# LeoIV/polyaxon

Hardware: AMD Instinct MI355X
Metric: HPO trials/hour (whole node) + wall-clock-to-target, ResNet-50 Hyperband sweep (higher is better)
Workload: dtype bf16

## Files before the change

polyaxon_amd/csrc/bn_kernels.hip:

```cpp
#include <hip/hip_runtime.h>

#include "handoff.h"
#include <stdint.h>

#define PLX_API extern "C" __attribute__((visibility("default")))

namespace {

constexpr int kBlock = 256;

struct alignas(16) bf16x8 {
  uint16_t v[8];
};

__device__ __forceinline__ float bf2f(uint16_t b) { return __uint_as_float(((uint32_t)b) << 16); }

__device__ __forceinline__ uint16_t f2bf(float f) {
  return __builtin_bit_cast(uint16_t, (__bf16)f);
}

__device__ __forceinline__ void load8(const bf16x8* p, float* f) {
  const bf16x8 v = *p;
#pragma unroll
  for (int k = 0; k < 8; ++k) f[k] = bf2f(v.v[k]);
// ... 865 lines not shown
                                          int64_t M, int C, const float* gamma, const float* save_mean,
                                          const float* save_invstd, float* dgamma, float* dbeta, float* coef,
                                          const float* partials, int nblk, float* l2, int relu, int accumulate,
                                          const ResBn* resbn, unsigned* counters, hipStream_t stream) {
  Plan p;
  if (!plan_for(M, C, &p) || M < 1 || nblk < 1 || (relu && mask == nullptr)) return 1;
  if (resbn != nullptr && (dres == nullptr || resbn->part == nullptr)) return 1;
  const ResBn rb = resbn != nullptr ? *resbn : ResBn{};
  reduce_finalize_bwd(stream, partials, nblk, l2, counters,
                      BwdFin{C, M, gamma, save_mean, save_invstd, dgamma, dbeta, coef, accumulate});
  const int64_t n_vec = M * p.G;
  launch_dx(stream, n_vec, p.G, x, mask, dy, dx, dres, coef, relu, rb);
  return (int)hipGetLastError();
}

PLX_API int plx_stem_bn_pool_forward(const void* x, void* y, void* idx, int N, int H, int W, int C, const float* gamma,
                                     const float* beta, float eps, float momentum, float* running_mean,
                                     float* running_var, float* save_mean, float* save_invstd, float* scale_bias,
                                     float* partials, const float* ext_part, int ext_nblk, unsigned* counters,
                                     hipStream_t stream) {
  const int G = C / 8;
  if (N <= 0 || H <= 0 || W <= 0 || C % 8 || G > 256 || 256 % G) return 1;
  const int rc = ext_part != nullptr
                     ? plx_bn_forward_from_partials(x, nullptr, nullptr, (int64_t)N * H * W, C, gamma, beta, eps,
                                                    momentum, running_mean, running_var, save_mean, save_invstd,
                                                    scale_bias, ext_part, ext_nblk, partials, nullptr, 1, nullptr,
                                                    counters, stream)
                     : plx_bn_forward(x, nullptr, nullptr, (int64_t)N * H * W, C, gamma, beta, eps, momentum,
                                      running_mean, running_var, save_mean, save_invstd, scale_bias, partials, nullptr,
                                      1, nullptr, counters, stream);
// ... 35 lines not shown
```

polyaxon_amd/csrc/conv_gemm.hip:

```cpp
#include <hip/hip_runtime.h>

#include <stdint.h>

namespace {

typedef __bf16 bf16x8 __attribute__((ext_vector_type(8)));
typedef short s16x4 __attribute__((ext_vector_type(4)));
typedef float f32x4 __attribute__((ext_vector_type(4)));
typedef __attribute__((address_space(3))) void lds_void;
typedef __attribute__((address_space(1))) const void gbl_void;

constexpr int BK = 64;

struct ConvGeom {
    int H, W;
    int Hr, Wr;
    int C, S, ntaps;
    int Hc, Wc, OS, oph, opw;
    signed char offh[9], offw[9], btap[9];
    int tap_a[9], tap_b[9];
    uint32_t mWr, mHr;
    int nh, nw, hv[3], wv[3];
    uint32_t pat[9];
    int tap_inner;
// ... 25 lines not shown
    g.mWr = div_magic(g.Wr);
    g.mHr = div_magic(g.Hr);
    return g;
}

struct BnBwd {
    const __bf16* x;
    const uint8_t* mask;
    const float* mean;
    const float* invstd;
    float* part;
    int part_ld, blk_off;
    int skip_h, skip_w;
};

__device__ __forceinline__ void row_coords(int m, int Hr, int Wr, int& n, int& r, int& c) {
    const int q = m / Wr;
    c = m - q * Wr;
    n = q / Hr;
    r = q - n * Hr;
}

__device__ __forceinline__ void row_coords(int m, const ConvGeom& g, int& n, int& r, int& c) {
    const int q = g.mWr ? (int)__umulhi((uint32_t)m, g.mWr) : m;
    c = m - q * g.Wr;
    n = g.mHr ? (int)__umulhi((uint32_t)q, g.mHr) : q;
    r = q - n * g.Hr;
}

__device__ __forceinline__ size_t out_row(const ConvGeom& g, int m) {
// ... 27 lines not shown

__device__ __forceinline__ __amdgpu_buffer_rsrc_t buf_rsrc(const void* base) {
    return __builtin_amdgcn_make_buffer_rsrc(const_cast<void*>(base), 0, (int)OOB, 0x00020000);
}

__device__ __forceinline__ void blds16(__amdgpu_buffer_rsrc_t r, uint32_t off, void* l) {
    __builtin_amdgcn_raw_ptr_buffer_load_lds(r, (lds_void*)l, 16, off, 0, 0, 0);
}

__device__ __forceinline__ uint32_t pack_bf16x2(float a, float b) {
    return (uint32_t)__builtin_bit_cast(uint16_t, (__bf16)a) | ((uint32_t)__builtin_bit_cast(uint16_t, (__bf16)b) << 16);
}

__device__ __forceinline__ int nt_swz(int row) { return (row >> 1) & 7; }

template <int BM, int BN, int WGM, int WGN, int MODE, int MINB = 2, int NBUF = 2, bool BWD = false, int NTH = NTHREADS>
__global__ void __launch_bounds__(NTH, MINB)
gemm_nt_kernel(const __bf16* __restrict__ A, const __bf16* __restrict__ B, __bf16* __restrict__ C,
               int M, int N, int K, int lda, int ldb, int ldc, const __bf16* __restrict__ zero,
               float* __restrict__ stats, ConvGeom geo, const __bf16* __restrict__ D, int ldd, BnBwd bnr,
               const uint8_t* __restrict__ dmask) {
    constexpr bool CONV = MODE == 1, STEM = MODE == 2;
    static_assert(MODE >= 0 && MODE <= 2, "dense, gather or stem");
    constexpr int NW = NTH / 64;
    static_assert(WGM * WGN == NW, "one wave per wave tile");
    static_assert(NTH == 256 && NBUF >= 1 && NBUF <= 2, "4-wave kernels, one or two K stages");
    constexpr int WTM = BM / WGM, WTN = BN / WGN;
    constexpr int RM = WTM / 16, RN = WTN / 16;
    constexpr int A_BYTES = BM * BK * 2, B_BYTES = BN * BK * 2, STAGE = A_BYTES + B_BYTES;
    extern __shared__ __attribute__((aligned(16))) char smem[];

    const int tid = threadIdx.x, lane = tid & 63;
    const int wave = __builtin_amdgcn_readfirstlane(tid >> 6);
    const int ntn = N / BN, ntm = (M + BM - 1) / BM;
    const int id = xcd_remap(blockIdx.x, ntm * ntn);
    const int tn = id % ntn, tm = id / ntn;
    const int m0 = tm * BM, n0 = tn * BN;
    const int wm = wave / WGN, wn = wave % WGN;
// ... 83 lines not shown
#pragma unroll
        for (int b = 0; b < RM; ++b) acc[a][b] = f32x4{0.f, 0.f, 0.f, 0.f};

    const int fr = lane & 15, fq = lane >> 4;
    const int nk = K / BK;
    const int cdim = CONV ? geo.C : K;
    int st = 0, sc = 0;
    const bool tap_inner = CONV && geo.tap_inner;
    auto advance = [&]() {
        const bool wt = st + 1 == geo.ntaps, wc = sc + BK == cdim;
        const int st_i = wt ? 0 : st + 1, sc_i = wt ? sc + BK : sc;
        const int st_m = wc ? st + 1 : st, sc_m = wc ? 0 : sc + BK;
        st = tap_inner ? st_i : st_m;
        sc = tap_inner ? sc_i : sc_m;
    };
    stage(0, 0, 0, 0);
    advance();
    asm volatile("s_waitcnt vmcnt(0)" ::: "memory");
    __syncthreads();
    for (int kt = 0; kt < nk; ++kt) {
        const int cur = NBUF == 2 ? kt & 1 : 0;
        if (NBUF == 1 && kt > 0) {
            stage(0, kt * BK, st, sc);
            advance();
            asm volatile("s_waitcnt vmcnt(0)" ::: "memory");
            __syncthreads();
        }
        if (NBUF == 2 && kt + 1 < nk) {
            stage(cur ^ 1, (kt + 1) * BK, st, sc);
            advance();
        }
        const char* As = smem + cur * STAGE;
        const char* Bs = As + A_BYTES;
#pragma unroll
        for (int kk = 0; kk < 2; ++kk) {
            bf16x8 fa[RN], fb[RM];
#pragma unroll
            for (int rn = 0; rn < RN; ++rn) {
                const int row = wn * WTN + rn * 16 + fr;
                const int pc = (kk * 4 + fq) ^ nt_swz(row);
                fa[rn] = *(const bf16x8*)(Bs + row * 128 + pc * 16);
            }
#pragma unroll
            for (int rm = 0; rm < RM; ++rm) {
                const int row = wm * WTM + rm * 16 + fr;
                const int pc = (kk * 4 + fq) ^ nt_swz(row);
                fb[rm] = *(const bf16x8*)(As + row * 128 + pc * 16);
            }
#pragma unroll
            for (int rn = 0; rn < RN; ++rn)
#pragma unroll
                for (int rm = 0; rm < RM; ++rm)
                    acc[rn][rm] = __builtin_amdgcn_mfma_f32_16x16x32_bf16(fa[rn], fb[rm], acc[rn][rm], 0, 0, 0);
        }
        if (NBUF == 2) asm volatile("s_waitcnt vmcnt(0)" ::: "memory");
        __syncthreads();
    }
    constexpr int CROW = BN * 2 + 16;
    constexpr int CHUNKS = BN / 8;
    static_assert(NTH % CHUNKS == 0, "a thread keeps one chunk column over the store loop");
    constexpr int RSTEP = NTH / CHUNKS, ITERS = BM / RSTEP;
    const int rows = min(BM, M - m0);
    const int cc = tid % CHUNKS, r0 = tid / CHUNKS;
    const int ch0 = n0 + cc * 8;
    const bool bnr_on = BWD && bnr.part != nullptr;
    const bool stats_on = !BWD && stats != nullptr;
    const bool d_on = BWD && D != nullptr;
    int orow[ITERS];
#pragma unroll
    for (int it = 0; it < ITERS; ++it) {
        const int gm = min(m0 + r0 + it * RSTEP, M - 1);
// ... 619 lines not shown
    static_assert(NBUF >= 1 && NBUF <= 2, "one or two K stages");
    static_assert(NBUF == 1 || EPI <= KLOOP, "epilogue staging must fit the k-loop LDS");
    static_assert(LDS <= 160 * 1024, "LDS");
    constexpr int PER_CU = (160 * 1024) / LDS;
    constexpr int CAP = CONV != 0 && BN == 64 ? 3 : 4;
    constexpr int MIN_F = NBUF == 1 ? (PER_CU < CAP ? PER_CU : CAP) : 2, MIN_B = MIN_F;
    auto kf = gemm_nt_kernel<BM, BN, WGM, WGN, CONV, MIN_F, NBUF, false, NTH>;
    auto kb = gemm_nt_kernel<BM, BN, WGM, WGN, CONV, MIN_B, NBUF, true, NTH>;
    static int attr = set_lds(kf, LDS) | set_lds(kb, LDS);
    if (attr) return attr;
    const bool bwd = D != nullptr || bnr.part != nullptr;
    if (bwd && stats != nullptr) return -1;
    auto k = bwd ? kb : kf;
    const int nwg = ((M + BM - 1) / BM) * (N / BN);
    hipLaunchKernelGGL(k, dim3(nwg), dim3(NTH), LDS, s, (const __bf16*)A, (const __bf16*)B, (__bf16*)C, M, N,
                       K, lda, ldb, ldc, (const __bf16*)zero, stats, geo, (const __bf16*)D, ldd, bnr, dmask);
    return hipGetLastError() == hipSuccess ? 0 : -3;
}


inline bool nt_single(bool conv, int K, int nwg) { return nwg >= 768 || (!conv && K == BK); }

struct TnPlan { int kchunk, slices, groups, per_group, blocks, bn1, bn2; };

inline void tn_tile(int N1, int N2, int& bn1, int& bn2) {
    bn1 = N1 % 128 == 0 ? 128 : 64;
    bn2 = N2 % 128 == 0 ? 128 : 64;
}

constexpr int g_tn_blocks_per_cu = 0;
constexpr int g_tn_bpc_big = 3, g_tn_bpc_mid = 1;
// ... 187 lines not shown
    if (dmask != nullptr && (D == nullptr || ldd != N)) return -1;
    if (bnr != nullptr && (ldc != N || bnr->part == nullptr)) return -1;
    const BnBwd b = bnr != nullptr ? *bnr : BnBwd{};
    hipStream_t s = (hipStream_t)stream;
    if (N % 128 == 0) {
        const bool one = nt_single(false, K, ((M + 127) / 128) * (N / 128));
        return one ? launch_nt<128, 128, 2, 2, false, 1>(A, B, C, M, N, K, lda, ldb, ldc, zero, stats, s, {}, D, ldd, b,
                                                         dmask)
                   : launch_nt<128, 128, 2, 2>(A, B, C, M, N, K, lda, ldb, ldc, zero, stats, s, {}, D, ldd, b, dmask);
    }
    const bool one = nt_single(false, K, ((M + 255) / 256) * (N / 64));
    return one ? launch_nt<256, 64, 4, 1, false, 1>(A, B, C, M, N, K, lda, ldb, ldc, zero, stats, s, {}, D, ldd, b, dmask)
               : launch_nt<256, 64, 4, 1>(A, B, C, M, N, K, lda, ldb, ldc, zero, stats, s, {}, D, ldd, b, dmask);
}

int plx_tn_plan_slices(int M, int N1, int N2, int num_cus, int v2) {
    if (M <= 0 || N1 % 64 || N2 % 64) return -1;
    return v2 ? tn2_plan(M, N1, N2, num_cus, v2_cfg(N1, N2)).slices : tn_plan(M, N1, N2, num_cus).slices;
}

void plx_set_tn2_c64(int on) { g_tn2_c64 = on ? 1 : 0; }

void plx_set_tn_atomic(int on) { g_tn_atomic = on ? 1 : 0; }

void plx_set_tn2_stem(int mode) { g_tn2_stem = mode < 0 ? 0 : (mode > 2 ? 2 : mode); }

void plx_set_tn_v2(int on, int lds_kb) {
    g_tn_v2 = on < 0 ? 0 : (on > 2 ? 2 : on);
    if (lds_kb > 0) g_tn2_lds_kb = lds_kb <= 64 ? 64 : 128;
}
// ... 374 lines not shown
```

polyaxon_amd/ops/_native.py:

```python
from __future__ import annotations

import ctypes
import hashlib
import os
import shutil
import subprocess
import threading
from pathlib import Path
from typing import Dict, Iterable, List, Optional

PKG_DIR = Path(__file__).resolve().parent.parent
CSRC = PKG_DIR / "csrc"
OUT = PKG_DIR / "_native"
ARCH = os.environ.get("PLX_OFFLOAD_ARCH", "gfx950")
ROCM = Path(os.environ.get("ROCM_PATH", "/opt/rocm"))

LIBRARIES: Dict[str, dict] = {
    "plx_train": {"sources": ["train_kernels.hip"], "kind": "hip", "link": []},
    "plx_polytune": {"sources": ["polytune_kernels.hip"], "kind": "hip", "link": []},
    "plx_bn": {"sources": ["bn_kernels.hip"], "kind": "hip", "link": []},
    "plx_procmon": {"sources": ["procmon.cpp"], "kind": "cpp", "link": ["-lpthread"]},
    "plx_gp": {"sources": ["gp_kernels.hip", "gp_chol.hip"], "kind": "hip", "link": []},
    "plx_rms": {"sources": ["rmsnorm.hip"], "kind": "hip", "link": []},
    "plx_conv": {"sources": ["conv_gemm.hip"], "kind": "hip", "link": []},
# ... 164 lines not shown
        "plx_synth_images": [_P, _P, _I, _I, _I, _P, _I, _I, _F, _U64, _P, _P],
        "plx_set_adamw_grid_cap": [_I],
        "plx_set_adamw_wide": [_I],
    },
    "plx_bn": {
        "plx_bn_workspace": [_L, _I],
        "plx_bn_forward": [_P, _P, _P, _L, _I, _P, _P, _F, _F, _P, _P, _P, _P, _P, _P, _P, _I, _P, _P, _P],
        "plx_bn_apply": [_P, _P, _P, _L, _I, _P, _I, _P],
        "plx_bn_l2_workspace": [_I, _I],
        "plx_bn_forward_from_partials": [_P, _P, _P, _L, _I, _P, _P, _F, _F, _P, _P, _P, _P, _P, _P, _I, _P, _P,
                                         _I, _P, _P, _P],
        "plx_bn_backward": [_P, _P, _P, _P, _P, _L, _I, _P, _P, _P, _P, _P, _P, _P, _I, _I, _P, _P, _P],
        "plx_bn_dx_blocks": [_L, _I],
        "plx_bn_backward_from_partials": [_P, _P, _P, _P, _P, _L, _I, _P, _P, _P, _P, _P, _P, _P, _I, _P, _I, _I, _P,
                                          _P, _P],
        "plx_stem_bn_pool_forward": [_P, _P, _P, _I, _I, _I, _I, _P, _P, _F, _F, _P, _P, _P, _P, _P, _P, _P, _I, _P,
                                     _P],
        "plx_stem_bn_pool_bwd_workspace": [_I, _I, _I, _I],
        "plx_stem_bn_pool_backward": [_P, _P, _P, _P, _I, _I, _I, _I, _P, _P, _P, _P, _P, _P, _P, _P, _I, _P, _P],
    },
    "plx_procmon": {
        "plx_pm_create": [],
        "plx_pm_destroy": [_P],
        "plx_pm_spawn": [_P, _P, _P, ctypes.c_char_p, ctypes.c_char_p, ctypes.POINTER(_I)],
        "plx_pm_wait": [_P, _I, ctypes.POINTER(_I), ctypes.POINTER(_I)],
        "plx_pm_wake": [_P],
        "plx_pm_signal": [_P, _I, _I, _I],
        "plx_pm_count": [_P],
    },
    "plx_gp": {
        "plx_gp_kmat": [_P, _P, _I, _I, _I, _P, _I, _I, _F, _F, _F, _I, _F, _P, _P, _D, _I, _P],
        "plx_gp_chol": [_P, _I, _I, _P, _P],
        "plx_gp_kmat_batch_f64": [_P, _I, _I, _P, _I, _P, _I, _L, _I, _D, _D, _D, _P, _P, _D, _I, _P],
        "plx_gp_matern_table": [_D, _D, _D, _I, _P, _P, _P],
        "plx_gp_chol_aug_f64": [_P, _I, _I, _I, _L, _I, _P, _P, _P],
        "plx_gp_chol_scratch_doubles": [],
        "plx_gp_lml_f64": [_P, _I, _I, _L, _I, _P, _P, _P],
        "plx_gp_acq_rows": [_P, _I, _I, _P, _F, _I, _F, _F, _F, _P, _P, _P, _P],
        "plx_gp_predict_acq": [_P, _I, _P, _I, _I, _P, _I, _P, _I, _F, _F, _F, _F, _I, _F, _F, _F, _P, _P, _P, _P,
                               _P, _P, _P, _D, _I, _P],
        "plx_gp_ascent": [_P, _P, _I, _P, _P, _P, _I, _I, _P, _P, _I, _F, _F, _F, _F, _I, _F, _F, _F, _I, _P, _P, _D, _I,
                          _P],
    },
    "plx_conv": {
        "plx_gemm_nt": [_P, _P, _P, _I, _I, _I, _I, _I, _I, _P, _P, _P, _I, _P, _P, _P],
        "plx_gemm_nt_rows_per_block": [_I],
        "plx_gemm_tn_workspace": [_I, _I, _I, _I],
        "plx_set_tn_v2": [_I, _I],
        "plx_set_tn2_stem": [_I],
        "plx_set_tn2_c64": [_I],
        "plx_set_tn_atomic": [_I],
        "plx_tn_plan_slices": [_I, _I, _I, _I, _I],
        "plx_gemm_tn": [_P, _P, _P, _P, _I, _I, _I, _I, _I, _I, _P, _I, _I, _P],
        "plx_weight_prep": [_P, _P, _P, _I, _I, _P],
        "plx_weight_prepk": [_P, _L, _L, _L, _L, _P, _P, _I, _I, _I, _P],
        "plx_weight_prep_all": [_P, _P, _P, _P, _I, _I, _P],
        "plx_stem_pack_input": [_P, _P, _I, _I, _I, _P],
        "plx_stem_pack_weight": [_P, _L, _L, _L, _L, _P, _I, _P],
        "plx_stem_conv_rows_per_block": [],
        "plx_stem_conv_fwd": [_P, _P, _P, _I, _I, _I, _P, _P, _P],
# ... 113 lines not shown
```

polyaxon_amd/ops/bn_fused.py:

```python
from __future__ import annotations

import ctypes

from typing import Optional

import torch

from polyaxon_amd.ops import _native
from polyaxon_amd.ops.conv1x1 import BnLink
from polyaxon_amd.ops.flat import direct_grad


def _stream() -> int:
    return _native.current_stream()


_COUNTERS = {}


def _counters(dev: torch.device):
    key = (dev.index, torch.cuda.current_stream(dev).cuda_stream)
    return _native.cached(_COUNTERS, key, lambda: torch.zeros(64, dtype=torch.int32, device=dev)).data_ptr()


def _cl(t: torch.Tensor) -> torch.Tensor:
    return t if t.is_contiguous(memory_format=torch.channels_last) else t.contiguous(memory_format=torch.channels_last)


def supported(x: torch.Tensor) -> bool:
    if not x.is_cuda or x.dtype != torch.bfloat16 or x.dim() != 4:
        return False
    c = x.shape[1]
    g = c // 8
    return c % 8 == 0 and g > 0 and (g & (g - 1)) == 0 and x.numel() > 0


class _BNAct(torch.autograd.Function):
    @staticmethod
    def forward(ctx, x, weight, bias, running_mean, running_var, residual, momentum, eps, relu, ext=None, box=None,
                link=None, rlink=None, defer=False):
        lib = _native.lib("plx_bn")
        x = _cl(x)
        n, c, h, w = x.shape
        m = n * h * w
        ws = _native.size("plx_bn", "plx_bn_workspace", m, c)
        if ws < 0:
            raise RuntimeError("unsupported channel count for fused BN")
        f32 = dict(dtype=torch.float32, device=x.device)
        defer = bool(defer) and not relu and residual is None and link is not None
        y = None if defer else torch.empty_like(x, memory_format=torch.channels_last)
        yp = y.data_ptr() if y is not None else None
        stats = torch.empty(4 * c, **f32)
        res_sb = None
        if residual is not None:
            rl = getattr(residual, "_plx_bn_link", None)
            if rl is not None and rl.affine is not None and getattr(residual, "_plx_deferred", False):
# ... 51 lines not shown
        if dy.dtype != torch.bfloat16:
            dy = dy.to(torch.bfloat16)
        f32 = dict(dtype=torch.float32, device=x.device)
        dx = torch.empty_like(x, memory_format=torch.channels_last)
        masked_box = ctx.box is not None and ctx.relu and mask is not None
        dres = (torch.empty_like(x, memory_format=torch.channels_last)
                if ctx.has_res and not masked_box else None)
        if ctx.direct is not None:
            dg_ptr, db_ptr, acc = ctx.direct[0].data_ptr(), ctx.direct[1].data_ptr(), 1
            dgb = None
        else:
            dgb = torch.empty(2 * c, **f32)
            dg_ptr, db_ptr, acc = dgb.data_ptr(), dgb[c:].data_ptr(), 0
        coef = torch.empty(3 * c, **f32)
        part, nblk = ctx.link.take() if ctx.link is not None else (None, 0)
        rb = None
        if ctx.rlink is not None and dres is not None:
            rl = ctx.rlink
            nblk2 = _native.size("plx_bn", "plx_bn_dx_blocks", m, c)
            rl.part = torch.empty(2 * nblk2 * c, **f32)
            rl.nblk = nblk2
            rb = _native.ResBnArgs(rl.x.data_ptr(), rl.mask.data_ptr() if rl.mask is not None else None,
                                   rl.mean.data_ptr(), rl.invstd.data_ptr(), rl.part.data_ptr())
        rbp = ctypes.addressof(rb) if rb is not None else None
        if part is not None:
            l2 = torch.empty(_native.size("plx_bn", "plx_bn_l2_workspace", nblk, c), **f32)
            rc = lib.plx_bn_backward_from_partials(
                x.data_ptr(), mask.data_ptr() if mask is not None else None, dy.data_ptr(), dx.data_ptr(),
                dres.data_ptr() if dres is not None else None, m, c, weight.data_ptr(), stats.data_ptr(),
                stats[c:].data_ptr(), dg_ptr, db_ptr, coef.data_ptr(), part.data_ptr(), nblk, l2.data_ptr(),
# ... 3 lines not shown
            partials = torch.empty(ctx.ws, **f32)
            rc = lib.plx_bn_backward(
                x.data_ptr(), mask.data_ptr() if mask is not None else None, dy.data_ptr(), dx.data_ptr(),
                dres.data_ptr() if dres is not None else None, m, c, weight.data_ptr(), stats.data_ptr(),
                stats[c:].data_ptr(), dg_ptr, db_ptr, coef.data_ptr(), partials.data_ptr(), int(ctx.relu), acc,
                rbp, _counters(x.device), _stream())
            _native.check(rc, "plx_bn_backward")
        if ctx.box is not None:
            if masked_box:
                ctx.box.put_masked(dy, mask)
            else:
                ctx.box.put(dres)
            dres = None
        dgamma = dgb[:c] if dgb is not None else None
        dbeta = dgb[c:] if dgb is not None else None
        return dx, dgamma, dbeta, None, None, dres, None, None, None, None, None, None, None, None


class _Materialize(torch.autograd.Function):

    @staticmethod
    def forward(ctx, t, sb):
        c = t.shape[1]
        return (t.float() * sb[:c].view(1, c, 1, 1) + sb[c:].view(1, c, 1, 1)).to(t.dtype).contiguous(
            memory_format=torch.channels_last)

    @staticmethod
    def backward(ctx, g):
        return g, None


def materialize(t: Optional[torch.Tensor]) -> Optional[torch.Tensor]:
    if t is None or not getattr(t, "_plx_deferred", False):
        return t
    return _Materialize.apply(t, t._plx_bn_link.affine)


def bn_act(x: torch.Tensor, weight: torch.Tensor, bias: torch.Tensor, running_mean: Optional[torch.Tensor],
           running_var: Optional[torch.Tensor], training: bool, momentum: float, eps: float,
           residual: Optional[torch.Tensor], act: bool, ext_stats=None, residual_grad_box=None,
           residual_link: bool = False, defer_apply: bool = False) -> torch.Tensor:
    if residual is not None and residual.dtype != x.dtype:
        residual = residual.to(x.dtype)
    if training:
        link = BnLink()
        rlink = getattr(residual, "_plx_bn_link", None) if (residual_link and residual is not None) else None
        defer = bool(defer_apply) and not act and residual is None
        y = _BNAct.apply(x, weight, bias, running_mean, running_var, residual, momentum, eps, act, ext_stats,
                         residual_grad_box, link, rlink, defer)
        y._plx_bn_link = link
        if defer:
            y._plx_deferred = True
        return y
    residual = materialize(residual)
    lib = _native.lib("plx_bn")
    x = _cl(x)
    n, c, h, w = x.shape
    inv = torch.rsqrt(running_var.float() + eps)
    scale = weight.float() * inv
    sb = torch.cat([scale, bias.float() - running_mean.float() * scale]).contiguous()
    y = torch.empty_like(x, memory_format=torch.channels_last)
    res = _cl(residual) if residual is not None else None
    rc = lib.plx_bn_apply(x.data_ptr(), res.data_ptr() if res is not None else None, y.data_ptr(), n * h * w, c,
                          sb.data_ptr(), int(act), _stream())
# ... 3 lines not shown
```

polyaxon_amd/ops/conv1x1.py:

```python
from __future__ import annotations

import ctypes
from typing import Dict

import torch
import torch.nn as nn
import torch.nn.functional as F

from polyaxon_amd.ops import _native, side_stream, wcache
from polyaxon_amd.ops.flat import direct_grad

_ZERO: Dict[int, torch.Tensor] = {}
_CUS: Dict[int, int] = {}


def _zero_page(dev: torch.device) -> torch.Tensor:
    idx = dev.index if dev.index is not None else torch.cuda.current_device()
    return _native.cached(_ZERO, idx, lambda: torch.zeros(256, dtype=torch.bfloat16, device=dev))


def _num_cus(dev: torch.device) -> int:
    idx = dev.index if dev.index is not None else torch.cuda.current_device()
    if idx not in _CUS:
        _CUS[idx] = torch.cuda.get_device_properties(idx).multi_processor_count
    return _CUS[idx]


def _stream() -> int:
# ... 18 lines not shown
    if add is not None:
        assert add.shape == (m, n) and add.stride(1) == 1 and add.dtype == torch.bfloat16 and add.data_ptr() % 16 == 0
    if add_mask is not None:
        assert add is not None and add.stride(0) == n and add_mask.dtype == torch.uint8 and add_mask.numel() == m * n // 8
    rc = _native.lib("plx_conv").plx_gemm_nt(a.data_ptr(), b.data_ptr(), out.data_ptr(), m, n, k, a.stride(0),
                                             b.stride(0), out.stride(0), _zero_page(a.device).data_ptr(),
                                             stats.data_ptr() if stats is not None else None,
                                             add.data_ptr() if add is not None else None,
                                             add.stride(0) if add is not None else 0,
                                             add_mask.data_ptr() if add_mask is not None else None,
                                             ctypes.addressof(bnr) if bnr is not None else None, _stream())
    _native.check(rc, "plx_gemm_nt")
    return out


def gemm_tn(a: torch.Tensor, b: torch.Tensor, out: torch.Tensor = None, accumulate: bool = False) -> torch.Tensor:
    m, n1 = a.shape
    n2 = b.shape[1]
    if out is None:
        out = torch.empty(n1, n2, dtype=torch.float32, device=a.device)
        accumulate = False
    assert a.stride(1) == 1 and b.stride(1) == 1 and out.stride(1) == 1 and b.shape[0] == m
    assert a.data_ptr() % 16 == 0 and b.data_ptr() % 16 == 0 and out.data_ptr() % 16 == 0
    lib = _native.lib("plx_conv")
    cus = _num_cus(a.device)
    ws = torch.empty(_native.size("plx_conv", "plx_gemm_tn_workspace", m, n1, n2, cus), dtype=torch.float32,
                     device=a.device)
    rc = lib.plx_gemm_tn(a.data_ptr(), b.data_ptr(), out.data_ptr(), ws.data_ptr(), m, n1, n2, a.stride(0),
                         b.stride(0), out.stride(0), _zero_page(a.device).data_ptr(), cus, int(accumulate),
                         _stream())
# ... 41 lines not shown
    def take(self):
        g, m = self.grad, self.mask
        self.grad = self.mask = None
        if g is None and self.expect:
            raise RuntimeError("GradMailbox: the deferred gradient did not arrive before its consumer's backward")
        return g, m


def unpack_relu_mask(g: torch.Tensor, mask: torch.Tensor) -> torch.Tensor:
    bits = (mask.view(-1, 1) >> torch.arange(8, device=mask.device, dtype=torch.uint8)) & 1
    n, c, h, w = g.shape
    keep = bits.view(n, h, w, c).permute(0, 3, 1, 2).to(g.dtype)
    return (g * keep).contiguous(memory_format=torch.channels_last)


class BnLink:

    __slots__ = ("x", "mask", "mean", "invstd", "part", "nblk", "_args", "affine", "split")

    def __init__(self, x=None, mask=None, mean=None, invstd=None):
        self.x, self.mask, self.mean, self.invstd = x, mask, mean, invstd
        self.affine = None
        self.part = None
        self.nblk = 0
        self._args = None
        self.split = 0

    def _args_for(self, nblk_total: int, blk_off: int) -> "_native.BnBwdArgs":
        return _native.BnBwdArgs(self.x.data_ptr(), self.mask.data_ptr() if self.mask is not None else None,
                                 self.mean.data_ptr(), self.invstd.data_ptr(), self.part.data_ptr(), nblk_total,
# ... 29 lines not shown
        return part, nblk


def _rows(t: torch.Tensor) -> torch.Tensor:
    n, c, h, w = t.shape
    return t.permute(0, 2, 3, 1).reshape(n * h * w, c)


def bn_link_of(x: torch.Tensor, want: bool):
    link = getattr(x, "_plx_bn_link", None) if want else None
    return link if (link is not None and link.x is not None and link.x.shape == x.shape) else None


class _Conv1x1(torch.autograd.Function):
    @staticmethod
    def forward(ctx, x, weight, stats, box, sink, link):
        x = x.to(torch.bfloat16).contiguous(memory_format=torch.channels_last)
        ctx.box = box
        ctx.sink = sink if (sink is not None and sink.armed) else None
        if ctx.sink is not None:
            ctx.sink.expect = True
        ctx.link = link if (sink is None or sink.armed) else None
        ctx.wgrad = direct_grad(weight)
        n, cin, h, w = x.shape
        cout = weight.shape[0]
        wb, wt = wcache.lookup(weight) or weight_prep(weight)
        y = torch.empty((n, cout, h, w), dtype=torch.bfloat16, device=x.device, memory_format=torch.channels_last)
        gemm_nt(_rows(x), wb, _rows(y), stats)
        ctx.save_for_backward(x, wt)
        ctx.wshape = weight.shape
        ctx.wdtype = weight.dtype
        return y

    @staticmethod
    def backward(ctx, dy):
        x, wt = ctx.saved_tensors
        n, cin, h, w = x.shape
        dy = dy.to(torch.bfloat16).contiguous(memory_format=torch.channels_last)
        dx = dw = None
        extra, extra_mask = ctx.box.take() if ctx.box is not None else (None, None)
        if ctx.needs_input_grad[0]:
            dx = torch.empty_like(x, memory_format=torch.channels_last)
            if extra is not None and (extra.dtype != torch.bfloat16
                                      or not extra.is_contiguous(memory_format=torch.channels_last)):
                if extra_mask is not None:
                    extra, extra_mask = unpack_relu_mask(extra, extra_mask), None
                extra = extra.to(torch.bfloat16).contiguous(memory_format=torch.channels_last)
            bnr = None
            rows = nt_stats_rows(cin)
            if ctx.link is not None and ctx.sink is None and (ctx.box is None or extra is not None):
                bnr = ctx.link.request(-(-(n * h * w) // rows))
            elif ctx.link is not None and ctx.sink is not None and ctx.sink.s2k1 and extra is None:
                bnr = ctx.link.request_split(-(-(n * h * w) // rows), -(-(n * ((h + 1) // 2) * ((w + 1) // 2)) // rows))
            gemm_nt(_rows(dy), wt, _rows(dx), add=_rows(extra) if extra is not None else None, bnr=bnr,
                    add_mask=extra_mask)
            if ctx.sink is not None:
                ctx.sink.put(dx)
                dx = None
        if ctx.needs_input_grad[1]:
            cout = ctx.wshape[0]
            if ctx.wgrad is not None:
                slot = ctx.wgrad.as_strided((cout, cin), (cin, 1))
                side_stream.run(lambda: gemm_tn(_rows(dy), _rows(x), out=slot, accumulate=True), (dy, x), x.device)
            else:
                dw = gemm_tn(_rows(dy), _rows(x)).view(ctx.wshape).to(ctx.wdtype)
        return dx, dw, None, None, None, None


def _bf16_context(x: torch.Tensor) -> bool:
    if x.dtype == torch.bfloat16:
        return True
    return torch.is_autocast_enabled("cuda") and torch.get_autocast_dtype("cuda") == torch.bfloat16


def supported(x: torch.Tensor, conv: nn.Conv2d) -> bool:
    return (x.is_cuda and x.dim() == 4 and _bf16_context(x) and conv.kernel_size == (1, 1) and conv.stride == (1, 1)
            and conv.padding == (0, 0) and conv.groups == 1 and conv.bias is None
            and conv.in_channels % 64 == 0 and conv.out_channels % 64 == 0 and x.numel() > 0)


def conv1x1(x: torch.Tensor, weight: torch.Tensor, with_stats: bool = False,
            grad_box: "GradMailbox" = None, grad_sink: "GradMailbox" = None, bn_link: bool = False) -> torch.Tensor:
    stats = None
    if with_stats:
        n, _, h, w = x.shape
        m, cout = n * h * w, weight.shape[0]
        nblk = -(-m // nt_stats_rows(cout))
        stats = torch.empty(2 * nblk * cout, dtype=torch.float32, device=x.device)
    if grad_box is not None:
        grad_box.armed = True
    y = _Conv1x1.apply(x, weight, stats, grad_box, grad_sink, bn_link_of(x, bn_link))
    if stats is not None:
        y._plx_channel_stats = (stats, nblk)
    return y


class Conv1x1(nn.Conv2d):

    def __init__(self, in_ch: int, out_ch: int, stride: int = 1, native: bool = True, bn_stats: bool = True):
        super().__init__(in_ch, out_ch, 1, stride=stride, bias=False)
        self.native = native
        self.bn_stats = bn_stats

    def forward(self, x: torch.Tensor, grad_box: GradMailbox = None, grad_sink: GradMailbox = None,
                bn_link: bool = False) -> torch.Tensor:
        if self.native and supported(x, self):
            return conv1x1(x, self.weight, with_stats=self.bn_stats and self.training, grad_box=grad_box,
                           grad_sink=grad_sink, bn_link=bn_link)
# ... 2 lines not shown
```

polyaxon_amd/ops/norm.py:

```python
from __future__ import annotations

from typing import Optional

import torch
import torch.nn as nn
import torch.nn.functional as F


def bn_act_reference(x: torch.Tensor, weight: torch.Tensor, bias: torch.Tensor,
                     running_mean: Optional[torch.Tensor], running_var: Optional[torch.Tensor],
                     training: bool, momentum: float, eps: float, residual: Optional[torch.Tensor],
                     act: bool) -> torch.Tensor:
    y = F.batch_norm(x, running_mean, running_var, weight, bias, training, momentum, eps)
    if residual is not None:
        y = y + residual
    if act:
        y = F.relu(y)
    return y


class BatchNormAct(nn.Module):
    def __init__(self, num_features: int, act: bool = True, residual: bool = False, fused: bool = True,
                 eps: float = 1e-5, momentum: float = 0.1):
        super().__init__()
# ... 11 lines not shown
    def reset_running_stats(self) -> None:
        with torch.no_grad():
            self.running_mean.zero_()
            self.running_var.fill_(1.0)

    def forward(self, x: torch.Tensor, identity: Optional[torch.Tensor] = None, residual_grad_box=None,
                residual_link: bool = False, defer_apply: bool = False) -> torch.Tensor:
        if self.residual and identity is None:
            raise ValueError("BatchNormAct(residual=True) needs the identity tensor")
        if self.fused and x.is_cuda:
            from polyaxon_amd.ops import bn_fused
            if bn_fused.supported(x):
                ext = getattr(x, "_plx_channel_stats", None)
                return bn_fused.bn_act(x, self.weight, self.bias, self.running_mean, self.running_var,
                                       self.training, self.momentum, self.eps, identity, self.act, ext,
                                       residual_grad_box, residual_link, defer_apply)
        if identity is not None and identity.is_cuda:
            from polyaxon_amd.ops.bn_fused import materialize
            identity = materialize(identity)
        return bn_act_reference(x, self.weight, self.bias, self.running_mean, self.running_var,
                                self.training, self.momentum, self.eps, identity, self.act)

    def extra_repr(self) -> str:
        return f"{self.num_features}, act={self.act}, residual={self.residual}, fused={self.fused}"
```

Before: 12400.

## Fuse BatchNorm input-gradient apply into the following 1x1 conv data-gradient GEMM

```diff
diff --git a/polyaxon_amd/csrc/bn_kernels.hip b/polyaxon_amd/csrc/bn_kernels.hip
--- a/polyaxon_amd/csrc/bn_kernels.hip
+++ b/polyaxon_amd/csrc/bn_kernels.hip
@@ -903,6 +903,33 @@
   return (int)hipGetLastError();
 }
 
+PLX_API int plx_bn_backward_coef(const void* x, const uint8_t* mask, const void* dy, int64_t M, int C,
+                                 const float* gamma, const float* save_mean, const float* save_invstd, float* dgamma,
+                                 float* dbeta, float* coef, float* partials, int relu, int accumulate,
+                                 unsigned* counters, hipStream_t stream) {
+  Plan p;
+  if (!plan_for(M, C, &p) || M < 1 || (relu && mask == nullptr)) return 1;
+  float* pa = partials;
+  float* pb = partials + (int64_t)p.nblk * C;
+  hipLaunchKernelGGL(relu ? bn_bwd_reduce_kernel<true> : bn_bwd_reduce_kernel<false>, dim3(p.nblk, p.gy), dim3(kBlock), 0, stream, (const bf16x8*)x,
+                     mask, (const bf16x8*)dy, M, p.G, p.Gb, p.rows_per_block, save_mean, save_invstd,
+                     relu, pa, pb);
+  reduce_finalize_bwd(stream, partials, p.nblk, partials + 2 * (int64_t)p.nblk * C, counters,
+                      BwdFin{C, M, gamma, save_mean, save_invstd, dgamma, dbeta, coef, accumulate});
+  return (int)hipGetLastError();
+}
+
+PLX_API int plx_bn_backward_coef_from_partials(int64_t M, int C, const float* gamma, const float* save_mean,
+                                               const float* save_invstd, float* dgamma, float* dbeta, float* coef,
+                                               const float* partials, int nblk, float* l2, int accumulate,
+                                               unsigned* counters, hipStream_t stream) {
+  Plan p;
+  if (!plan_for(M, C, &p) || M < 1 || nblk < 1) return 1;
+  reduce_finalize_bwd(stream, partials, nblk, l2, counters,
+                      BwdFin{C, M, gamma, save_mean, save_invstd, dgamma, dbeta, coef, accumulate});
+  return (int)hipGetLastError();
+}
+
 PLX_API int plx_stem_bn_pool_forward(const void* x, void* y, void* idx, int N, int H, int W, int C, const float* gamma,
                                      const float* beta, float eps, float momentum, float* running_mean,
                                      float* running_var, float* save_mean, float* save_invstd, float* scale_bias,
diff --git a/polyaxon_amd/csrc/conv_gemm.hip b/polyaxon_amd/csrc/conv_gemm.hip
--- a/polyaxon_amd/csrc/conv_gemm.hip
+++ b/polyaxon_amd/csrc/conv_gemm.hip
@@ -7,6 +7,7 @@
 typedef __bf16 bf16x8 __attribute__((ext_vector_type(8)));
 typedef short s16x4 __attribute__((ext_vector_type(4)));
 typedef float f32x4 __attribute__((ext_vector_type(4)));
+typedef uint32_t u32x4 __attribute__((ext_vector_type(4)));
 typedef __attribute__((address_space(3))) void lds_void;
 typedef __attribute__((address_space(1))) const void gbl_void;
 
@@ -63,6 +64,13 @@
     int skip_h, skip_w;
 };
 
+struct BnDx {
+    const __bf16* x;
+    const uint8_t* mask;
+    const float* coef;
+    __bf16* dy;
+};
+
 __device__ __forceinline__ void row_coords(int m, int Hr, int Wr, int& n, int& r, int& c) {
     const int q = m / Wr;
     c = m - q * Wr;
@@ -120,14 +128,16 @@
 
 __device__ __forceinline__ int nt_swz(int row) { return (row >> 1) & 7; }
 
-template <int BM, int BN, int WGM, int WGN, int MODE, int MINB = 2, int NBUF = 2, bool BWD = false, int NTH = NTHREADS>
+template <int BM, int BN, int WGM, int WGN, int MODE, int MINB = 2, int NBUF = 2, bool BWD = false, int NTH = NTHREADS,
+          bool BNDX = false>
 __global__ void __launch_bounds__(NTH, MINB)
 gemm_nt_kernel(const __bf16* __restrict__ A, const __bf16* __restrict__ B, __bf16* __restrict__ C,
                int M, int N, int K, int lda, int ldb, int ldc, const __bf16* __restrict__ zero,
                float* __restrict__ stats, ConvGeom geo, const __bf16* __restrict__ D, int ldd, BnBwd bnr,
-               const uint8_t* __restrict__ dmask) {
+               const uint8_t* __restrict__ dmask, BnDx bd) {
     constexpr bool CONV = MODE == 1, STEM = MODE == 2;
     static_assert(MODE >= 0 && MODE <= 2, "dense, gather or stem");
+    static_assert(!BNDX || (MODE == 0 && NBUF == 2 && BWD && NTH == 256), "BNDX: dense double-buffered data gradient");
     constexpr int NW = NTH / 64;
     static_assert(WGM * WGN == NW, "one wave per wave tile");
     static_assert(NTH == 256 && NBUF >= 1 && NBUF <= 2, "4-wave kernels, one or two K stages");
@@ -241,19 +251,101 @@
         st = tap_inner ? st_i : st_m;
         sc = tap_inner ? sc_i : sc_m;
     };
-    stage(0, 0, 0, 0);
-    advance();
-    asm volatile("s_waitcnt vmcnt(0)" ::: "memory");
-    __syncthreads();
+    constexpr int XI = BNDX ? AI : 1;
+    uint32_t e_off[XI];
+    u32x4 gq[XI], xq[XI], oq[XI];
+    uint32_t mq[XI];
+    u32x4 cf[6];
+    const int lc8 = (((lane & 7) ^ nt_swz(wave * 8 + (lane >> 3))) & 7) * 8;
+    const bool dy_owner = tn == 0;
+    if constexpr (BNDX) {
+#pragma unroll
+        for (int i = 0; i < XI; ++i) {
+            const int gm = m0 + (i * NW + wave) * 8 + (lane >> 3);
+            e_off[i] = gm < M ? (uint32_t)((gm * K + lc8) * 2) : OOB;
+        }
+    }
+    auto load_a = [&](int k0) {
+        const __amdgpu_buffer_rsrc_t rx = buf_rsrc(bd.x), rc = buf_rsrc(bd.coef);
+#pragma unroll
+        for (int i = 0; i < XI; ++i) {
+            gq[i] = __builtin_amdgcn_raw_buffer_load_b128(ra, (int)e_off[i], k0 * 2, 0);
+            xq[i] = __builtin_amdgcn_raw_buffer_load_b128(rx, (int)e_off[i], k0 * 2, 0);
+        }
+        if (bd.mask != nullptr) {
+            const __amdgpu_buffer_rsrc_t rm = buf_rsrc(bd.mask);
+#pragma unroll
+            for (int i = 0; i < XI; ++i)
+                mq[i] = __builtin_amdgcn_raw_buffer_load_b8(rm, (int)(e_off[i] == OOB ? OOB : e_off[i] >> 4), k0 >> 3, 0);
+        } else {
+#pragma unroll
+            for (int i = 0; i < XI; ++i) mq[i] = 0xffu;
+        }
+#pragma unroll
+        for (int r = 0; r < 3; ++r) {
+            cf[2 * r] = __builtin_amdgcn_raw_buffer_load_b128(rc, lc8 * 4, (r * K + k0) * 4, 0);
+            cf[2 * r + 1] = __builtin_amdgcn_raw_buffer_load_b128(rc, lc8 * 4 + 16, (r * K + k0) * 4, 0);
+        }
+    };
+    auto xform_a = [&](int buf) {
+        char* base = smem + buf * STAGE;
+        const float* ca = (const float*)&cf[0];
+        const float* cb = (const float*)&cf[2];
+        const float* cd = (const float*)&cf[4];
+#pragma unroll
+        for (int i = 0; i < XI; ++i) {
+            const uint32_t* pg = (const uint32_t*)&gq[i];
+            const uint32_t* px = (const uint32_t*)&xq[i];
+            uint32_t* po = (uint32_t*)&oq[i];
+            const uint32_t mb = mq[i];
+#pragma unroll
+            for (int j = 0; j < 4; ++j) {
+                const float g0 = (mb >> (2 * j)) & 1u ? __uint_as_float(pg[j] << 16) : 0.f;
+                const float g1 = (mb >> (2 * j + 1)) & 1u ? __uint_as_float(pg[j] & 0xffff0000u) : 0.f;
+                const float x0 = __uint_as_float(px[j] << 16), x1 = __uint_as_float(px[j] & 0xffff0000u);
+                const float o0 = fmaf(ca[2 * j], g0, fmaf(cb[2 * j], x0, cd[2 * j]));
+                const float o1 = fmaf(ca[2 * j + 1], g1, fmaf(cb[2 * j + 1], x1, cd[2 * j + 1]));
+                po[j] = pack_bf16x2(o0, o1);
+            }
+            if (e_off[i] == OOB) oq[i] = u32x4{0u, 0u, 0u, 0u};
+            *(u32x4*)(base + (i * NW + wave) * 1024 + lane * 16) = oq[i];
+        }
+    };
+    auto store_dy = [&](int k0) {
+        if (!dy_owner) return;
+        const __amdgpu_buffer_rsrc_t rd = buf_rsrc(bd.dy);
+#pragma unroll
+        for (int i = 0; i < XI; ++i) __builtin_amdgcn_raw_buffer_store_b128(oq[i], rd, (int)e_off[i], k0 * 2, 0);
+    };
+    if constexpr (BNDX) {
+        static_assert(!BNDX || NW == 4, "a thread's rows step by 32: one chunk column per thread");
+        load_a(0);
+        stage_b(0, 0, 0, 0);
+        xform_a(0);
+        asm volatile("s_waitcnt vmcnt(0)" ::: "memory");
+        __syncthreads();
+        store_dy(0);
+    } else {
+        stage(0, 0, 0, 0);
+        advance();
+        asm volatile("s_waitcnt vmcnt(0)" ::: "memory");
+        __syncthreads();
+    }
     for (int kt = 0; kt < nk; ++kt) {
         const int cur = NBUF == 2 ? kt & 1 : 0;
-        if (NBUF == 1 && kt > 0) {
+        if constexpr (BNDX) {
+            if (kt + 1 < nk) {
+                load_a((kt + 1) * BK);
+                stage_b(cur ^ 1, (kt + 1) * BK, 0, 0);
+            }
+        }
+        if (!BNDX && NBUF == 1 && kt > 0) {
             stage(0, kt * BK, st, sc);
             advance();
             asm volatile("s_waitcnt vmcnt(0)" ::: "memory");
             __syncthreads();
         }
-        if (NBUF == 2 && kt + 1 < nk) {
+        if (!BNDX && NBUF == 2 && kt + 1 < nk) {
             stage(cur ^ 1, (kt + 1) * BK, st, sc);
             advance();
         }
@@ -280,8 +372,14 @@
                 for (int rm = 0; rm < RM; ++rm)
                     acc[rn][rm] = __builtin_amdgcn_mfma_f32_16x16x32_bf16(fa[rn], fb[rm], acc[rn][rm], 0, 0, 0);
         }
+        if constexpr (BNDX) {
+            if (kt + 1 < nk) xform_a(cur ^ 1);
+        }
         if (NBUF == 2) asm volatile("s_waitcnt vmcnt(0)" ::: "memory");
         __syncthreads();
+        if constexpr (BNDX) {
+            if (kt + 1 < nk) store_dy((kt + 1) * BK);
+        }
     }
     constexpr int CROW = BN * 2 + 16;
     constexpr int CHUNKS = BN / 8;
@@ -931,7 +1029,23 @@
     auto k = bwd ? kb : kf;
     const int nwg = ((M + BM - 1) / BM) * (N / BN);
     hipLaunchKernelGGL(k, dim3(nwg), dim3(NTH), LDS, s, (const __bf16*)A, (const __bf16*)B, (__bf16*)C, M, N,
-                       K, lda, ldb, ldc, (const __bf16*)zero, stats, geo, (const __bf16*)D, ldd, bnr, dmask);
+                       K, lda, ldb, ldc, (const __bf16*)zero, stats, geo, (const __bf16*)D, ldd, bnr, dmask, BnDx{});
+    return hipGetLastError() == hipSuccess ? 0 : -3;
+}
+
+template <int BM, int BN, int WGM, int WGN>
+int launch_nt_bndx(const void* g, const BnDx& bd, const void* B, void* C, int M, int N, int K, int ldb, int ldc,
+                   hipStream_t s, const void* D, int ldd, BnBwd bnr, const uint8_t* dmask) {
+    constexpr int TILE = BM * (BN * 2 + 16), RED = NTHREADS * 17 * 4;
+    constexpr int LDS = 2 * (BM + BN) * BK * 2;
+    static_assert(TILE <= LDS && RED <= LDS && LDS <= 80 * 1024, "epilogue staging fits; 2 blocks per CU");
+    auto k = gemm_nt_kernel<BM, BN, WGM, WGN, 0, 2, 2, true, NTHREADS, true>;
+    static int attr = set_lds(k, LDS);
+    if (attr) return attr;
+    const int nwg = ((M + BM - 1) / BM) * (N / BN);
+    hipLaunchKernelGGL(k, dim3(nwg), dim3(NTHREADS), LDS, s, (const __bf16*)g, (const __bf16*)B, (__bf16*)C, M, N, K, K,
+                       ldb, ldc, (const __bf16*)nullptr, (float*)nullptr, ConvGeom{}, (const __bf16*)D, ldd, bnr, dmask,
+                       bd);
     return hipGetLastError() == hipSuccess ? 0 : -3;
 }
 
@@ -1149,6 +1263,21 @@
                : launch_nt<256, 64, 4, 1>(A, B, C, M, N, K, lda, ldb, ldc, zero, stats, s, {}, D, ldd, b, dmask);
 }
 
+int plx_gemm_nt_bndx(const void* g, const void* x, const uint8_t* mask, const float* coef, void* dy, const void* Wt,
+                     void* C, int M, int N, int K, int ldb, int ldc, const void* D, int ldd, const uint8_t* dmask,
+                     const BnBwd* bnr, void* stream) {
+    if (M <= 0 || N % 64 || K % BK || ldb % 8 || ldc % 8 || (D != nullptr && ldd % 8)) return -1;
+    if (g == nullptr || x == nullptr || coef == nullptr || dy == nullptr || dy == g || dy == x) return -1;
+    if ((long)M * K >= (1l << 30)) return -1;
+    if (dmask != nullptr && (D == nullptr || ldd != N)) return -1;
+    if (bnr != nullptr && (ldc != N || bnr->part == nullptr)) return -1;
+    const BnBwd b = bnr != nullptr ? *bnr : BnBwd{};
+    const BnDx bd{(const __bf16*)x, mask, coef, (__bf16*)dy};
+    hipStream_t s = (hipStream_t)stream;
+    if (N % 128 == 0) return launch_nt_bndx<128, 128, 2, 2>(g, bd, Wt, C, M, N, K, ldb, ldc, s, D, ldd, b, dmask);
+    return launch_nt_bndx<256, 64, 4, 1>(g, bd, Wt, C, M, N, K, ldb, ldc, s, D, ldd, b, dmask);
+}
+
 int plx_tn_plan_slices(int M, int N1, int N2, int num_cus, int v2) {
     if (M <= 0 || N1 % 64 || N2 % 64) return -1;
     return v2 ? tn2_plan(M, N1, N2, num_cus, v2_cfg(N1, N2)).slices : tn_plan(M, N1, N2, num_cus).slices;
diff --git a/polyaxon_amd/ops/_native.py b/polyaxon_amd/ops/_native.py
--- a/polyaxon_amd/ops/_native.py
+++ b/polyaxon_amd/ops/_native.py
@@ -202,6 +202,8 @@
         "plx_bn_dx_blocks": [_L, _I],
         "plx_bn_backward_from_partials": [_P, _P, _P, _P, _P, _L, _I, _P, _P, _P, _P, _P, _P, _P, _I, _P, _I, _I, _P,
                                           _P, _P],
+        "plx_bn_backward_coef": [_P, _P, _P, _L, _I, _P, _P, _P, _P, _P, _P, _P, _I, _I, _P, _P],
+        "plx_bn_backward_coef_from_partials": [_L, _I, _P, _P, _P, _P, _P, _P, _P, _I, _P, _I, _P, _P],
         "plx_stem_bn_pool_forward": [_P, _P, _P, _I, _I, _I, _I, _P, _P, _F, _F, _P, _P, _P, _P, _P, _P, _P, _I, _P,
                                      _P],
         "plx_stem_bn_pool_bwd_workspace": [_I, _I, _I, _I],
@@ -232,6 +234,7 @@
     },
     "plx_conv": {
         "plx_gemm_nt": [_P, _P, _P, _I, _I, _I, _I, _I, _I, _P, _P, _P, _I, _P, _P, _P],
+        "plx_gemm_nt_bndx": [_P, _P, _P, _P, _P, _P, _P, _I, _I, _I, _I, _I, _P, _I, _P, _P, _P],
         "plx_gemm_nt_rows_per_block": [_I],
         "plx_gemm_tn_workspace": [_I, _I, _I, _I],
         "plx_set_tn_v2": [_I, _I],
diff --git a/polyaxon_amd/ops/bn_fused.py b/polyaxon_amd/ops/bn_fused.py
--- a/polyaxon_amd/ops/bn_fused.py
+++ b/polyaxon_amd/ops/bn_fused.py
@@ -38,8 +38,9 @@
 class _BNAct(torch.autograd.Function):
     @staticmethod
     def forward(ctx, x, weight, bias, running_mean, running_var, residual, momentum, eps, relu, ext=None, box=None,
-                link=None, rlink=None, defer=False):
+                link=None, rlink=None, defer=False, dxsink=None):
         lib = _native.lib("plx_bn")
+        ctx.dxsink = dxsink if x.is_contiguous(memory_format=torch.channels_last) else None
         x = _cl(x)
         n, c, h, w = x.shape
         m = n * h * w
@@ -121,6 +122,26 @@
             dg_ptr, db_ptr, acc = dgb.data_ptr(), dgb[c:].data_ptr(), 0
         coef = torch.empty(3 * c, **f32)
         part, nblk = ctx.link.take() if ctx.link is not None else (None, 0)
+        if ctx.dxsink is not None and dres is None:
+            if part is not None:
+                l2 = torch.empty(_native.size("plx_bn", "plx_bn_l2_workspace", nblk, c), **f32)
+                rc = lib.plx_bn_backward_coef_from_partials(
+                    m, c, weight.data_ptr(), stats.data_ptr(), stats[c:].data_ptr(), dg_ptr, db_ptr, coef.data_ptr(),
+                    part.data_ptr(), nblk, l2.data_ptr(), acc, _counters(x.device), _stream())
+                _native.check(rc, "plx_bn_backward_coef_from_partials")
+            else:
+                partials = torch.empty(ctx.ws, **f32)
+                rc = lib.plx_bn_backward_coef(
+                    x.data_ptr(), mask.data_ptr() if mask is not None else None, dy.data_ptr(), m, c,
+                    weight.data_ptr(), stats.data_ptr(), stats[c:].data_ptr(), dg_ptr, db_ptr, coef.data_ptr(),
+                    partials.data_ptr(), int(ctx.relu), acc, _counters(x.device), _stream())
+                _native.check(rc, "plx_bn_backward_coef")
+            ctx.dxsink.put(dy, x, mask if ctx.relu else None, coef, dx)
+            if ctx.box is not None:
+                ctx.box.put_masked(dy, mask)
+            dgamma = dgb[:c] if dgb is not None else None
+            dbeta = dgb[c:] if dgb is not None else None
+            return dx, dgamma, dbeta, None, None, None, None, None, None, None, None, None, None, None, None
         rb = None
         if ctx.rlink is not None and dres is not None:
             rl = ctx.rlink
@@ -154,7 +175,7 @@
             dres = None
         dgamma = dgb[:c] if dgb is not None else None
         dbeta = dgb[c:] if dgb is not None else None
-        return dx, dgamma, dbeta, None, None, dres, None, None, None, None, None, None, None, None
+        return dx, dgamma, dbeta, None, None, dres, None, None, None, None, None, None, None, None, None
 
 
 class _Materialize(torch.autograd.Function):
@@ -179,7 +200,7 @@
 def bn_act(x: torch.Tensor, weight: torch.Tensor, bias: torch.Tensor, running_mean: Optional[torch.Tensor],
            running_var: Optional[torch.Tensor], training: bool, momentum: float, eps: float,
            residual: Optional[torch.Tensor], act: bool, ext_stats=None, residual_grad_box=None,
-           residual_link: bool = False, defer_apply: bool = False) -> torch.Tensor:
+           residual_link: bool = False, defer_apply: bool = False, dx_sink=None) -> torch.Tensor:
     if residual is not None and residual.dtype != x.dtype:
         residual = residual.to(x.dtype)
     if training:
@@ -187,7 +208,7 @@
         rlink = getattr(residual, "_plx_bn_link", None) if (residual_link and residual is not None) else None
         defer = bool(defer_apply) and not act and residual is None
         y = _BNAct.apply(x, weight, bias, running_mean, running_var, residual, momentum, eps, act, ext_stats,
-                         residual_grad_box, link, rlink, defer)
+                         residual_grad_box, link, rlink, defer, dx_sink)
         y._plx_bn_link = link
         if defer:
             y._plx_deferred = True
diff --git a/polyaxon_amd/ops/conv1x1.py b/polyaxon_amd/ops/conv1x1.py
--- a/polyaxon_amd/ops/conv1x1.py
+++ b/polyaxon_amd/ops/conv1x1.py
@@ -1,6 +1,7 @@
 from __future__ import annotations
 
 import ctypes
+import os
 from typing import Dict
 
 import torch
@@ -12,6 +13,14 @@
 
 _ZERO: Dict[int, torch.Tensor] = {}
 _CUS: Dict[int, int] = {}
+
+_BN_DX_FUSED = os.environ.get("PLX_BN_DX_FUSED", "1") != "0"
+
+
+def set_bn_dx_fused(on: bool) -> bool:
+    global _BN_DX_FUSED
+    prev, _BN_DX_FUSED = _BN_DX_FUSED, bool(on)
+    return prev
 
 
 def _zero_page(dev: torch.device) -> torch.Tensor:
@@ -60,6 +69,35 @@
     return out
 
 
+def gemm_nt_bndx(g: torch.Tensor, x: torch.Tensor, mask: torch.Tensor, coef: torch.Tensor, dy: torch.Tensor,
+                 b: torch.Tensor, out: torch.Tensor = None, add: torch.Tensor = None,
+                 bnr: "_native.BnBwdArgs" = None, add_mask: torch.Tensor = None) -> torch.Tensor:
+    m, k = g.shape
+    n = b.shape[0]
+    if out is None:
+        out = torch.empty(m, n, dtype=torch.bfloat16, device=g.device)
+    for t in (g, x, dy):
+        assert t.shape == (m, k) and t.dtype == torch.bfloat16 and t.stride() == (k, 1) and t.data_ptr() % 16 == 0
+    assert b.stride(1) == 1 and out.stride(1) == 1 and b.shape[1] == k and b.dtype == torch.bfloat16
+    assert b.data_ptr() % 16 == 0 and out.data_ptr() % 16 == 0
+    assert coef.dtype == torch.float32 and coef.is_contiguous() and coef.numel() == 3 * k
+    if mask is not None:
+        assert mask.dtype == torch.uint8 and mask.numel() == m * k // 8
+    if add is not None:
+        assert add.shape == (m, n) and add.stride(1) == 1 and add.dtype == torch.bfloat16 and add.data_ptr() % 16 == 0
+    if add_mask is not None:
+        assert add is not None and add.stride(0) == n and add_mask.dtype == torch.uint8 and add_mask.numel() == m * n // 8
+    rc = _native.lib("plx_conv").plx_gemm_nt_bndx(g.data_ptr(), x.data_ptr(),
+                                                  mask.data_ptr() if mask is not None else None, coef.data_ptr(),
+                                                  dy.data_ptr(), b.data_ptr(), out.data_ptr(), m, n, k, b.stride(0),
+                                                  out.stride(0), add.data_ptr() if add is not None else None,
+                                                  add.stride(0) if add is not None else 0,
+                                                  add_mask.data_ptr() if add_mask is not None else None,
+                                                  ctypes.addressof(bnr) if bnr is not None else None, _stream())
+    _native.check(rc, "plx_gemm_nt_bndx")
+    return out
+
+
 def gemm_tn(a: torch.Tensor, b: torch.Tensor, out: torch.Tensor = None, accumulate: bool = False) -> torch.Tensor:
     m, n1 = a.shape
     n2 = b.shape[1]
@@ -131,6 +169,28 @@
     return (g * keep).contiguous(memory_format=torch.channels_last)
 
 
+class DxSink:
+
+    __slots__ = ("payload",)
+
+    def __init__(self):
+        self.payload = None
+
+    def put(self, g: torch.Tensor, x: torch.Tensor, mask, coef: torch.Tensor, dx: torch.Tensor) -> None:
+        self.payload = (g, x, mask, coef, dx)
+
+    def take(self):
+        p, self.payload = self.payload, None
+        return p
+
+
+def dx_sink_for(x: torch.Tensor, weight: torch.Tensor):
+    if not _BN_DX_FUSED or not (torch.is_grad_enabled() and x.requires_grad):
+        return None
+    cout, cin = weight.shape[0], weight.shape[1]
+    return DxSink() if (cout >= 2 * cin and cin <= 128) else None
+
+
 class BnLink:
 
     __slots__ = ("x", "mask", "mean", "invstd", "part", "nblk", "_args", "affine", "split")
@@ -190,9 +250,10 @@
 
 class _Conv1x1(torch.autograd.Function):
     @staticmethod
-    def forward(ctx, x, weight, stats, box, sink, link):
+    def forward(ctx, x, weight, stats, box, sink, link, dxsink=None):
         x = x.to(torch.bfloat16).contiguous(memory_format=torch.channels_last)
         ctx.box = box
+        ctx.dxsink = dxsink
         ctx.sink = sink if (sink is not None and sink.armed) else None
         if ctx.sink is not None:
             ctx.sink.expect = True
@@ -212,6 +273,11 @@
     def backward(ctx, dy):
         x, wt = ctx.saved_tensors
         n, cin, h, w = x.shape
+        fused = ctx.dxsink.take() if ctx.dxsink is not None else None
+        if fused is not None and (dy.data_ptr() != fused[4].data_ptr() or dy.shape != fused[4].shape
+                                  or dy.dtype != torch.bfloat16 or not ctx.needs_input_grad[0]):
+            raise RuntimeError("DxSink: the BatchNorm's deferred input gradient was replaced before the convolution's "
+                               "backward could fill it")
         dy = dy.to(torch.bfloat16).contiguous(memory_format=torch.channels_last)
         dx = dw = None
         extra, extra_mask = ctx.box.take() if ctx.box is not None else (None, None)
@@ -228,8 +294,13 @@
                 bnr = ctx.link.request(-(-(n * h * w) // rows))
             elif ctx.link is not None and ctx.sink is not None and ctx.sink.s2k1 and extra is None:
                 bnr = ctx.link.request_split(-(-(n * h * w) // rows), -(-(n * ((h + 1) // 2) * ((w + 1) // 2)) // rows))
-            gemm_nt(_rows(dy), wt, _rows(dx), add=_rows(extra) if extra is not None else None, bnr=bnr,
-                    add_mask=extra_mask)
+            if fused is not None:
+                g, bx, bmask, coef, _ = fused
+                gemm_nt_bndx(_rows(g), _rows(bx), bmask, coef, _rows(dy), wt, _rows(dx),
+                             add=_rows(extra) if extra is not None else None, bnr=bnr, add_mask=extra_mask)
+            else:
+                gemm_nt(_rows(dy), wt, _rows(dx), add=_rows(extra) if extra is not None else None, bnr=bnr,
+                        add_mask=extra_mask)
             if ctx.sink is not None:
                 ctx.sink.put(dx)
                 dx = None
@@ -240,7 +311,7 @@
                 side_stream.run(lambda: gemm_tn(_rows(dy), _rows(x), out=slot, accumulate=True), (dy, x), x.device)
             else:
                 dw = gemm_tn(_rows(dy), _rows(x)).view(ctx.wshape).to(ctx.wdtype)
-        return dx, dw, None, None, None, None
+        return dx, dw, None, None, None, None, None
 
 
 def _bf16_context(x: torch.Tensor) -> bool:
@@ -265,9 +336,12 @@
         stats = torch.empty(2 * nblk * cout, dtype=torch.float32, device=x.device)
     if grad_box is not None:
         grad_box.armed = True
-    y = _Conv1x1.apply(x, weight, stats, grad_box, grad_sink, bn_link_of(x, bn_link))
+    dxsink = dx_sink_for(x, weight)
+    y = _Conv1x1.apply(x, weight, stats, grad_box, grad_sink, bn_link_of(x, bn_link), dxsink)
     if stats is not None:
         y._plx_channel_stats = (stats, nblk)
+    if dxsink is not None:
+        y._plx_dx_sink = dxsink
     return y
 
 
diff --git a/polyaxon_amd/ops/norm.py b/polyaxon_amd/ops/norm.py
--- a/polyaxon_amd/ops/norm.py
+++ b/polyaxon_amd/ops/norm.py
@@ -49,7 +49,8 @@
                 ext = getattr(x, "_plx_channel_stats", None)
                 return bn_fused.bn_act(x, self.weight, self.bias, self.running_mean, self.running_var,
                                        self.training, self.momentum, self.eps, identity, self.act, ext,
-                                       residual_grad_box, residual_link, defer_apply)
+                                       residual_grad_box, residual_link, defer_apply,
+                                       getattr(x, "_plx_dx_sink", None))
         if identity is not None and identity.is_cuda:
             from polyaxon_amd.ops.bn_fused import materialize
             identity = materialize(identity)
```

Measured after the change: 12670 (median of 6 runs). 1.02x the previous value.
